# Jun-CEN/Open-World-Semantic-Segmentation

Hardware: AMD Instinct MI355X
Metric: images/sec train-step, DeepLabV3+R101 768x768 bs=16; % HBM & MFMA roofline (higher is better)
Workload: dtype f16x2

## Files before the change

open-world-semantic-segmentation_amd/csrc/bn.hip:

```cpp
#include "common.h"
#include <cstdlib>

namespace {

struct Moments {
    double n, mean, m2;
};
__device__ __forceinline__ void merge(Moments& a, double nb, double meanb, double m2b) {
    if (nb <= 0.0) return;
    const double n = a.n + nb;
    const double d = meanb - a.mean;
    a.mean += d * (nb / n);
    a.m2 += m2b + d * d * (a.n * nb / n);
    a.n = n;
}

constexpr int FIN_CH = 4, FIN_SL = 64;
__device__ __forceinline__ double shfl_xor_f64(double v, int mask) {
    const long long b = __double_as_longlong(v);
    const int lo = __shfl_xor((int)(b & 0xffffffffll), mask), hi = __shfl_xor((int)(b >> 32), mask);
    return __longlong_as_double(((long long)hi << 32) | (unsigned int)lo);
}

__device__ __forceinline__ float h2_words_max(const float* __restrict__ words, float* sh4) {
// ... 1202 lines not shown
#pragma unroll
                for (int t = 0; t < 2; ++t) {
                    const int s = 2 * bx + t - (2 * xo - 1);
                    if (s < 0 || s > 2) continue;
#pragma unroll
                    for (int q = 0; q < 4; ++q) acc[u][t][q] += (((am >> (q * 8)) & 0xffu) == (uint32_t)(r * 3 + s)) ? g[q] : 0.f;
                }
            }
        }
    }
#pragma unroll
    for (int u = 0; u < 2; ++u) {
#pragma unroll
        for (int t = 0; t < 2; ++t) {
            const int yi = 2 * by + u, xi = 2 * bx + t;
            if (yi >= H || xi >= W) continue;
            const uint32_t bits = mask[(((int64_t)b * H + yi) * W + xi) * (C / 4) + cv];
#pragma unroll
            for (int q = 0; q < 4; ++q) acc[u][t][q] = ((bits >> q) & 1u) != 0 ? acc[u][t][q] : 0.f;
        }
    }
}

__device__ __forceinline__ void stem_pixel_grad(const float* __restrict__ dp, const uint8_t* __restrict__ argmax, uint32_t bits, int b,
                                                int yi, int xi, int C, int Ho, int Wo, int cv, float (&acc)[4]) {
#pragma unroll
    for (int q = 0; q < 4; ++q) acc[q] = 0.f;
    const int by = yi >> 1, bx = xi >> 1, u = yi & 1, t = xi & 1;
#pragma unroll
    for (int dyo = 0; dyo < 2; ++dyo) {
        const int yo = by + dyo, r = u + 1 - 2 * dyo;
        if (yo >= Ho || r < 0) continue;
#pragma unroll
        for (int dxo = 0; dxo < 2; ++dxo) {
            const int xo = bx + dxo, sc = t + 1 - 2 * dxo;
            if (xo >= Wo || sc < 0) continue;
            const int64_t o = (((int64_t)b * Ho + yo) * Wo + xo) * C + cv * 4;
            float g[4];
            Vec16<float>::load(dp + o, g);
            const uint32_t am = *reinterpret_cast<const uint32_t*>(argmax + o);
#pragma unroll
            for (int q = 0; q < 4; ++q) acc[q] += (((am >> (q * 8)) & 0xffu) == (uint32_t)(r * 3 + sc)) ? g[q] : 0.f;
        }
    }
#pragma unroll
    for (int q = 0; q < 4; ++q) acc[q] = ((bits >> q) & 1u) != 0 ? acc[q] : 0.f;
}

__global__ __launch_bounds__(256) void stem_bwd_reduce_kernel(
    const float* __restrict__ dp, const uint8_t* __restrict__ argmax, const uint8_t* __restrict__ mask, const float* __restrict__ y,
    const float* __restrict__ save_mean, const float* __restrict__ save_invstd, float* __restrict__ partials, int B, int H, int W,
    int C, int ldy, int Ho, int Wo, int rows_per_block, int chv, int rt, uint32_t* __restrict__ gmax) {
    __shared__ float sh[256 * 2 * 4];
    uint32_t gmx = 0;
    const int NV = C / 4;
    const int64_t M = (int64_t)B * H * W;
    const int col = threadIdx.x % chv, rl = threadIdx.x / chv;
    const int v = blockIdx.y * chv + col;
    const bool active = rl < rt && v < NV;
    float sg[4], sgx[4];
#pragma unroll
    for (int q = 0; q < 4; ++q) { sg[q] = 0.f; sgx[q] = 0.f; }
    if (active) {
        const int c = v * 4;
        float mu[4], is[4];
#pragma unroll
        for (int q = 0; q < 4; ++q) { mu[q] = save_mean[c + q]; is[q] = save_invstd[c + q]; }
        const int64_t r0 = (int64_t)blockIdx.x * rows_per_block;
        const int64_t r1 = min(M, r0 + rows_per_block);
        constexpr int U = 2;
        for (int64_t m0 = r0 + rl; m0 < r1; m0 += (int64_t)rt * U) {
            float g[U][4], yy[U][4];
#pragma unroll
            for (int u = 0; u < U; ++u) {
                const int64_t m = m0 + (int64_t)u * rt;
                if (m < r1) {
                    const int xi = (int)(m % W), yi = (int)((m / W) % H), b = (int)(m / ((int64_t)W * H));
                    Vec16<float>::load(y + m * ldy + c, yy[u]);
                    stem_pixel_grad(dp, argmax, mask[m * NV + v], b, yi, xi, C, Ho, Wo, v, g[u]);
                }
            }
#pragma unroll
            for (int u = 0; u < U; ++u) {
                const int64_t m = m0 + (int64_t)u * rt;
                if (m >= r1) continue;
#pragma unroll
                for (int q = 0; q < 4; ++q) {
                    const float gg = g[u][q];
                    gmx = max(gmx, __float_as_uint(gg) & 0x7fffffffu);
                    sg[q] += gg;
                    sgx[q] += gg * (yy[u][q] - mu[q]) * is[q];
                }
            }
        }
    }
#pragma unroll
    for (int q = 0; q < 4; ++q) {
        sh[(threadIdx.x * 4 + q) * 2] = sg[q];
        sh[(threadIdx.x * 4 + q) * 2 + 1] = sgx[q];
    }
    __syncthreads();
    if (rl == 0 && v < NV) {
        for (int r = 1; r < rt; ++r) {
            const int t = r * chv + col;
// ... 144 lines not shown
#pragma unroll
        for (int q = 0; q < 4; ++q) wr[k][q] = k < K ? w[(int64_t)k * ldw + c + q] : 0.f;
    }
}
template <int KP>
__device__ __forceinline__ void head_load_de(const float* __restrict__ de_row, float (&d)[KP]) {
#pragma unroll
    for (int k = 0; k < KP; k += 4) {
        const float4 t = *reinterpret_cast<const float4*>(de_row + k);
        d[k] = t.x; d[k + 1] = t.y; d[k + 2] = t.z; d[k + 3] = t.w;
    }
}
template <int KP>
__device__ __forceinline__ void head_dz(const float (&d)[KP], const float (&wr)[KP][4], float (&g)[4]) {
#pragma unroll
    for (int q = 0; q < 4; ++q) {
        float a = 0.f;
#pragma unroll
        for (int k = 0; k < KP; ++k) a = fmaf(d[k], wr[k][q], a);
        g[q] = a;
    }
}

template <int KP>
__global__ __launch_bounds__(256) void head_bwd_reduce_kernel(
    const float* __restrict__ de, const float* __restrict__ w, const float* __restrict__ y, const uint8_t* __restrict__ mask,
    const float* __restrict__ save_mean, const float* __restrict__ save_invstd, float* __restrict__ partials, int64_t M, int N,
    int K, int ldde, int ldw, int ldy, int relu, int rows_per_block, int chv, int rt, uint32_t* __restrict__ gmax) {
    __shared__ float sh[256 * 2 * 4];
    uint32_t gmx = 0;
    const int NV = N / 4;
    const int col = threadIdx.x % chv, rl = threadIdx.x / chv;
    const int v = blockIdx.y * chv + col;
    const bool active = rl < rt && v < NV;
    float sg[4], sgx[4];
#pragma unroll
    for (int q = 0; q < 4; ++q) { sg[q] = 0.f; sgx[q] = 0.f; }
    if (active) {
        const int c = v * 4;
        float mu[4], is[4], wr[KP][4];
#pragma unroll
        for (int q = 0; q < 4; ++q) { mu[q] = save_mean[c + q]; is[q] = save_invstd[c + q]; }
        head_load_w<KP>(w, K, ldw, c, wr);
        const int64_t r0 = (int64_t)blockIdx.x * rows_per_block;
        const int64_t r1 = min(M, r0 + rows_per_block);
        constexpr int U = 2;
        for (int64_t m0 = r0 + rl; m0 < r1; m0 += (int64_t)rt * U) {
            float d[U][KP], yy[U][4];
            uint32_t bits[U];
#pragma unroll
            for (int u = 0; u < U; ++u) {
                const int64_t m = m0 + (int64_t)u * rt;
                bits[u] = 0xfu;
                if (m < r1) {
                    head_load_de<KP>(de + m * ldde, d[u]);
// ... 19 lines not shown
    }
#pragma unroll
    for (int q = 0; q < 4; ++q) {
        sh[(threadIdx.x * 4 + q) * 2] = sg[q];
        sh[(threadIdx.x * 4 + q) * 2 + 1] = sgx[q];
    }
    __syncthreads();
    if (rl == 0 && v < NV) {
        for (int r = 1; r < rt; ++r) {
            const int t = r * chv + col;
#pragma unroll
            for (int q = 0; q < 4; ++q) {
                sg[q] += sh[(t * 4 + q) * 2];
                sgx[q] += sh[(t * 4 + q) * 2 + 1];
            }
        }
        float* p = partials + ((int64_t)blockIdx.x * N + v * 4) * 2;
#pragma unroll
        for (int q = 0; q < 4; ++q) { p[2 * q] = sg[q]; p[2 * q + 1] = sgx[q]; }
    }
    if (gmax != nullptr) amax_publish(gmx, gmax);
}

template <int KP, int U, bool PAIR>
__global__ __launch_bounds__(64) void head_bwd_apply_kernel(
    const float* __restrict__ de, const float* __restrict__ w, const float* __restrict__ y, const uint8_t* __restrict__ mask,
    const float* __restrict__ coef, float* __restrict__ dy, int64_t M, int N, int K, int ldde, int ldw, int ldy, int lddy, int relu,
    int CB, int RB, int rows_per_block, _Float16* __restrict__ planes, int64_t plane_stride, int ldp,
    const float* __restrict__ unscale) {
    typedef _Float16 h4 __attribute__((ext_vector_type(4)));
    const float h2s = planes != nullptr ? 1.0f / unscale[0] : 1.0f;
    const int NV = N / 4;
    const int col = threadIdx.x % CB, rl = threadIdx.x / CB;
    const int vcol = blockIdx.y * CB + col;
    if (!(rl < RB && vcol < NV)) return;
    const int c = vcol * 4;
    float cA[4], cB[4], cC[4], cM[4], wr[KP][4];
#pragma unroll
    for (int q = 0; q < 4; ++q) {
        cA[q] = coef[c + q];
        cB[q] = coef[N + c + q];
        cC[q] = coef[2 * N + c + q];
        cM[q] = coef[3 * N + c + q];
    }
    head_load_w<KP>(w, K, ldw, c, wr);
    const int64_t r0 = (int64_t)blockIdx.x * rows_per_block;
    const int64_t r1 = min(M, r0 + rows_per_block);
    for (int64_t m0 = r0 + rl; m0 < r1; m0 += (int64_t)RB * U) {
        float d[U][KP], yy[U][4];
        uint32_t bits[U];
#pragma unroll
        for (int u = 0; u < U; ++u) {
            const int64_t m = m0 + (int64_t)u * RB;
            bits[u] = 0xfu;
            if (m < r1) {
                head_load_de<KP>(de + m * ldde, d[u]);
// ... 44 lines not shown
        return DML_EALIGN;
    if (M >= (1ll << 31)) return DML_EINVAL;
    return 0;
}
}

extern "C" int dml_head_bn_bwd_reduce(const void* de, const float* w, const void* y, const uint8_t* mask, const float* save_mean,
                                      const float* save_invstd, float* partials, int64_t M, int N, int K, int Kp, int ldde, int ldw,
                                      int ldy, int relu, int* nblocks, float* gmax, void* stream) {
    if (const int rc = head_bwd_args(de, w, y, mask, M, N, K, Kp, ldde, ldw, ldy, relu)) return rc;
    if (!save_mean || !save_invstd || !partials || !nblocks) return DML_EINVAL;
    const int NV = N / 4;
    const int chv = NV < RED_COLS ? NV : RED_COLS;
    const int rt = 256 / chv;
    const int col_chunks = (NV + chv - 1) / chv;
    int64_t rpb = (M * col_chunks + 1023) / 1024;
    if (rpb < 4 * rt) rpb = 4 * rt;
    rpb = ((rpb + rt - 1) / rt) * rt;
    const int rb = (int)((M + rpb - 1) / rpb);
    *nblocks = rb;
    const dim3 grid(rb, col_chunks);
    hipStream_t st = static_cast<hipStream_t>(stream);
#define DML_HEAD_REDUCE(KP)                                                                                                       \
    hipLaunchKernelGGL(head_bwd_reduce_kernel<KP>, grid, dim3(256), 0, st, (const float*)de, w, (const float*)y, mask, save_mean, \
                       save_invstd, partials, M, N, K, ldde, ldw, ldy, relu, (int)rpb, chv, rt, reinterpret_cast<uint32_t*>(gmax))
    if (Kp == 8) DML_HEAD_REDUCE(8);
    else if (Kp == 16) DML_HEAD_REDUCE(16);
    else if (Kp == 24) DML_HEAD_REDUCE(24);
    else DML_HEAD_REDUCE(32);
#undef DML_HEAD_REDUCE
    DML_LAUNCH_CHECK();
    return 0;
}

extern "C" int dml_head_bn_bwd_apply(const void* de, const float* w, const void* y, const uint8_t* mask, const float* coef, void* dy,
                                     int64_t M, int N, int K, int Kp, int ldde, int ldw, int ldy, int lddy, int relu, void* planes,
                                     int64_t plane_stride, int32_t ldp, const float* unscale, void* stream) {
    if (const int rc = head_bwd_args(de, w, y, mask, M, N, K, Kp, ldde, ldw, ldy, relu)) return rc;
    if (!coef || (!dy && !planes)) return DML_EINVAL;
    if (dy && ((lddy & 3) || lddy < N || (reinterpret_cast<uintptr_t>(dy) & 15))) return DML_EALIGN;
    if (planes) {
        if (!unscale || plane_stride <= 0 || ldp < N) return DML_EINVAL;
        if ((ldp & 3) || (plane_stride & 3) || (reinterpret_cast<uintptr_t>(planes) & 7)) return DML_EALIGN;
    }
    constexpr int bt = 64;
    const ColGeom g = col_geom(M, N / 4, 2, stream_blocks(M, N, DML_F32), bt);
    const dim3 grid(g.row_blocks, g.col_chunks);
    hipStream_t st = static_cast<hipStream_t>(stream);
    const bool pair = planes && !dy && (N & 7) == 0 && (ldp & 7) == 0 && (plane_stride & 7) == 0 &&
                      (reinterpret_cast<uintptr_t>(planes) & 15) == 0;
#define DML_HEAD_APPLY(KP, PAIR)                                                                                                   \
    hipLaunchKernelGGL((head_bwd_apply_kernel<KP, 2, PAIR>), grid, dim3(bt), 0, st, (const float*)de, w, (const float*)y, mask, coef, \
                       (float*)dy, M, N, K, ldde, ldw, ldy, lddy, relu, g.CB, g.RB, g.rows_per_block,                              \
                       static_cast<_Float16*>(planes), plane_stride, (int)ldp, unscale)
    if (pair) {
        if (Kp == 8) DML_HEAD_APPLY(8, true);
        else if (Kp == 16) DML_HEAD_APPLY(16, true);
        else if (Kp == 24) DML_HEAD_APPLY(24, true);
        else DML_HEAD_APPLY(32, true);
    } else {
        if (Kp == 8) DML_HEAD_APPLY(8, false);
        else if (Kp == 16) DML_HEAD_APPLY(16, false);
        else if (Kp == 24) DML_HEAD_APPLY(24, false);
        else DML_HEAD_APPLY(32, false);
    }
#undef DML_HEAD_APPLY
    DML_LAUNCH_CHECK();
    return 0;
}

namespace {
__global__ __launch_bounds__(256) void h2_bound_kernel(const float* __restrict__ p0, const float* __restrict__ p1,
                                                       const float* __restrict__ p2, const float* __restrict__ invstd, int N,
                                                       float root_count, float mult, const float* __restrict__ words,
                                                       float* __restrict__ work, int bwd) {
    __shared__ float sh[4];
    __shared__ uint32_t shw[4];
// ... 114 lines not shown
```

open-world-semantic-segmentation_amd/csrc/optim_layout.hip:

```cpp
#include "common.h"

namespace {

__global__ __launch_bounds__(256) void sgd_kernel(float* __restrict__ p, const float* __restrict__ g,
                                                  float* __restrict__ v, int64_t n, float lr, float mu, float wd,
                                                  float gscale) {
    const int64_t n4 = n >> 2;
    for (int64_t i = (int64_t)blockIdx.x * blockDim.x + threadIdx.x; i < n4;
         i += (int64_t)gridDim.x * blockDim.x) {
        float4 pp = reinterpret_cast<float4*>(p)[i];
        const float4 gg = reinterpret_cast<const float4*>(g)[i];
        float4 vv = reinterpret_cast<float4*>(v)[i];
        vv.x = mu * vv.x + (gscale * gg.x + wd * pp.x);
        vv.y = mu * vv.y + (gscale * gg.y + wd * pp.y);
        vv.z = mu * vv.z + (gscale * gg.z + wd * pp.z);
        vv.w = mu * vv.w + (gscale * gg.w + wd * pp.w);
        pp.x -= lr * vv.x; pp.y -= lr * vv.y; pp.z -= lr * vv.z; pp.w -= lr * vv.w;
        reinterpret_cast<float4*>(v)[i] = vv;
        reinterpret_cast<float4*>(p)[i] = pp;
    }
    const int64_t base = n4 << 2;
    const int64_t t = base + (int64_t)blockIdx.x * blockDim.x + threadIdx.x;
    if (t < n) {
        const float d = gscale * g[t] + wd * p[t];
// ... 373 lines not shown
    if (!table_device || count <= 0) return DML_EINVAL;
    hipStream_t st = static_cast<hipStream_t>(stream);
    hipLaunchKernelGGL(h2_amax_table_kernel, dim3(H2_TABLE_BLK, count), dim3(256), 0, st, table_device);
    hipLaunchKernelGGL(h2_split_table_kernel, dim3(H2_TABLE_BLK, count), dim3(256), 0, st, table_device);
    DML_LAUNCH_CHECK();
    return 0;
}

namespace {
__global__ __launch_bounds__(256) void pack_input_s2d_kernel(const float* __restrict__ x, float* __restrict__ y, int B, int C, int H, int W) {
    const int H2 = H >> 1, W2 = W >> 1, C4 = 4 * C;
    const int64_t total = (int64_t)B * H2 * W2;
    for (int64_t i = (int64_t)blockIdx.x * blockDim.x + threadIdx.x; i < total; i += (int64_t)gridDim.x * blockDim.x) {
        const int64_t b = i / ((int64_t)H2 * W2);
        const int64_t rem = i - b * H2 * W2;
        const int y2 = (int)(rem / W2), x2 = (int)(rem - (int64_t)y2 * W2);
        float* o = y + i * C4;
        for (int c = 0; c < C; ++c) {
            const float* src = x + ((b * C + c) * H + 2 * y2) * W + 2 * x2;
            o[c] = src[0]; o[C + c] = src[1]; o[2 * C + c] = src[W]; o[3 * C + c] = src[W + 1];
        }
    }
}
template <bool TO_S2D>
__global__ __launch_bounds__(256) void s2d_weights_kernel(float* __restrict__ w, float* __restrict__ w2, int N, int k, int C) {
    const int k2 = (k + 1) / 2, C4 = 4 * C, off = 2 * (((k - 1) / 2 + 1) / 2) - (k - 1) / 2;
    const int total = N * k2 * k2 * C4;
    for (int i = blockIdx.x * blockDim.x + threadIdx.x; i < total; i += gridDim.x * blockDim.x) {
        const int j = i % C4, s2 = (i / C4) % k2, r2 = (i / (C4 * k2)) % k2, n = i / (C4 * k2 * k2);
        const int c = j % C, dx = (j / C) & 1, dy = j / (2 * C);
        const int t = 2 * r2 + dy - off, u = 2 * s2 + dx - off;
        const bool in = t >= 0 && t < k && u >= 0 && u < k;
        const int wi = ((n * k + t) * k + u) * C + c;
        if (TO_S2D) w2[i] = in ? w[wi] : 0.f;
        else if (in) w[wi] += w2[i];
    }
}
}

namespace {
__global__ __launch_bounds__(256) void gather_taps_kernel(const float* __restrict__ src, float* __restrict__ dst, int rows, int taps_src,
                                                          int n, int ntaps, int t0, int t1, int t2, int t3) {
    const int n4 = n >> 2;
    const int64_t total = (int64_t)rows * ntaps * n4;
    for (int64_t i = (int64_t)blockIdx.x * blockDim.x + threadIdx.x; i < total; i += (int64_t)gridDim.x * blockDim.x) {
        const int v = (int)(i % n4), j = (int)((i / n4) % ntaps);
        const int64_t row = i / ((int64_t)n4 * ntaps);
        const int t = j == 0 ? t0 : (j == 1 ? t1 : (j == 2 ? t2 : t3));
        reinterpret_cast<float4*>(dst)[i] = reinterpret_cast<const float4*>(src)[(row * taps_src + t) * n4 + v];
    }
}
}

extern "C" int dml_gather_taps(const float* src, float* dst, int rows, int taps_src, int n, int ntaps, int t0, int t1, int t2, int t3,
                               void* stream) {
    if (!src || !dst || rows <= 0 || taps_src <= 0 || n <= 0 || ntaps <= 0 || ntaps > 4) return DML_EINVAL;
    const int t[4] = {t0, t1, t2, t3};
    for (int j = 0; j < ntaps; ++j)
        if (t[j] < 0 || t[j] >= taps_src) return DML_EINVAL;
    if ((n & 3) || ((reinterpret_cast<uintptr_t>(src) | reinterpret_cast<uintptr_t>(dst)) & 15)) return DML_EALIGN;
    hipLaunchKernelGGL(gather_taps_kernel, dim3(grid_for((int64_t)rows * ntaps * (n >> 2), 256, 256 * 16)), dim3(256), 0,
                       static_cast<hipStream_t>(stream), src, dst, rows, taps_src, n, ntaps, t0, t1, t2, t3);
    DML_LAUNCH_CHECK();
    return 0;
}

extern "C" int dml_pack_input_s2d(const float* x_nchw, float* y, int B, int C, int H, int W, void* stream) {
    if (!x_nchw || !y || B <= 0 || C <= 0 || H <= 0 || W <= 0) return DML_EINVAL;
    if ((H | W) & 1) return DML_EALIGN;
    hipLaunchKernelGGL(pack_input_s2d_kernel, dim3(grid_for((int64_t)B * (H / 2) * (W / 2), 256, 256 * 16)), dim3(256), 0,
                       static_cast<hipStream_t>(stream), x_nchw, y, B, C, H, W);
    DML_LAUNCH_CHECK();
    return 0;
}
extern "C" int dml_s2d_weights(const float* w, float* w2, int N, int k, int C, void* stream) {
    if (!w || !w2 || N <= 0 || C <= 0 || k < 3 || (k & 1) == 0 || (((k - 1) / 2) & 1) == 0) return DML_EINVAL;
    const int k2 = (k + 1) / 2;
    hipLaunchKernelGGL(s2d_weights_kernel<true>, dim3(grid_for((int64_t)N * k2 * k2 * 4 * C, 256)), dim3(256), 0,
                       static_cast<hipStream_t>(stream), const_cast<float*>(w), w2, N, k, C);
    DML_LAUNCH_CHECK();
    return 0;
}
extern "C" int dml_s2d_wgrad(const float* dw2, float* dw, int N, int k, int C, void* stream) {
    if (!dw2 || !dw || N <= 0 || C <= 0 || k < 3 || (k & 1) == 0 || (((k - 1) / 2) & 1) == 0) return DML_EINVAL;
    const int k2 = (k + 1) / 2;
    hipLaunchKernelGGL(s2d_weights_kernel<false>, dim3(grid_for((int64_t)N * k2 * k2 * 4 * C, 256)), dim3(256), 0,
                       static_cast<hipStream_t>(stream), dw, const_cast<float*>(dw2), N, k, C);
    DML_LAUNCH_CHECK();
    return 0;
}

extern "C" int dml_unpad_wgrad(const float* src, float* dst, int N, int RS, int Cm, int Cp, void* stream) {
    if (!src || !dst || Cp < Cm) return DML_EINVAL;
    hipLaunchKernelGGL(unpad_wgrad_kernel, dim3(grid_for((int64_t)N * RS * Cm, 256)), dim3(256), 0,
// ... 63 lines not shown
```

open-world-semantic-segmentation_amd/csrc/pool_resize.hip:

```cpp
#include "common.h"

namespace {

template <typename T>
__global__ __launch_bounds__(256) void maxpool_fwd_kernel(const T* __restrict__ x, T* __restrict__ y,
                                                          uint8_t* __restrict__ argmax, int B, int H, int W,
                                                          int C, int Ho, int Wo) {
    constexpr int V = Vec16<T>::N;
    const int CV = C / V;
    const int64_t total = (int64_t)B * Ho * Wo * CV;
    for (int64_t i = (int64_t)blockIdx.x * blockDim.x + threadIdx.x; i < total;
         i += (int64_t)gridDim.x * blockDim.x) {
        const int cv = (int)(i % CV);
        int64_t p = i / CV;
        const int xo = (int)(p % Wo); p /= Wo;
        const int yo = (int)(p % Ho);
        const int b = (int)(p / Ho);
        float best[V];
        int idx[V];
#pragma unroll
        for (int q = 0; q < V; ++q) { best[q] = -INFINITY; idx[q] = -1; }
#pragma unroll
        for (int r = 0; r < 3; ++r) {
            const int yi = yo * 2 - 1 + r;
// ... 167 lines not shown
         i += (int64_t)gridDim.x * blockDim.x) {
        const int cv = (int)(i % CV);
        int64_t p = i / CV;
        const int X = (int)(p % W); p /= W;
        const int Y = (int)(p % H);
        const int b = (int)(p / H);
        const Lerp ly = src_index(Y, sy, h), lx = src_index(X, sx, w);
        const TI* base = x + (int64_t)b * h * w * ldx + cv * V;
        float o[V];
#pragma unroll
        for (int q = 0; q < V; ++q) {
            const float v00 = Elem<TI>::ld(base + ((int64_t)ly.i0 * w + lx.i0) * ldx + q);
            const float v01 = Elem<TI>::ld(base + ((int64_t)ly.i0 * w + lx.i1) * ldx + q);
            const float v10 = Elem<TI>::ld(base + ((int64_t)ly.i1 * w + lx.i0) * ldx + q);
            const float v11 = Elem<TI>::ld(base + ((int64_t)ly.i1 * w + lx.i1) * ldx + q);
            o[q] = ly.l0 * (lx.l0 * v00 + lx.l1 * v01) + ly.l1 * (lx.l0 * v10 + lx.l1 * v11);
        }
        TO* yp = y + (((int64_t)b * H + Y) * W + X) * ldy + cv * V;
#pragma unroll
        for (int q = 0; q < V; ++q) Elem<TO>::st(yp + q, o[q]);
    }
}

__global__ __launch_bounds__(256) void bilinear_fwd_planes_kernel(const float* __restrict__ x, _Float16* __restrict__ planes,
                                                                  int64_t plane_stride, int ldp, const float* __restrict__ unscale, int B,
                                                                  int h, int w, int H, int W, int C, int ldx, float sy, float sx) {
    typedef _Float16 h4 __attribute__((ext_vector_type(4)));
    const int CV = C / 4;
    const float s = 1.0f / unscale[0];
    const int64_t total = (int64_t)B * H * W * CV;
    for (int64_t i = (int64_t)blockIdx.x * blockDim.x + threadIdx.x; i < total; i += (int64_t)gridDim.x * blockDim.x) {
        const int cv = (int)(i % CV);
        int64_t p = i / CV;
        const int X = (int)(p % W); p /= W;
        const int Y = (int)(p % H);
        const int b = (int)(p / H);
        const Lerp ly = src_index(Y, sy, h), lx = src_index(X, sx, w);
        const float* base = x + (int64_t)b * h * w * ldx + cv * 4;
        const float4 v00 = *reinterpret_cast<const float4*>(base + ((int64_t)ly.i0 * w + lx.i0) * ldx);
        const float4 v01 = *reinterpret_cast<const float4*>(base + ((int64_t)ly.i0 * w + lx.i1) * ldx);
        const float4 v10 = *reinterpret_cast<const float4*>(base + ((int64_t)ly.i1 * w + lx.i0) * ldx);
        const float4 v11 = *reinterpret_cast<const float4*>(base + ((int64_t)ly.i1 * w + lx.i1) * ldx);
        const float a00[4] = {v00.x, v00.y, v00.z, v00.w}, a01[4] = {v01.x, v01.y, v01.z, v01.w};
        const float a10[4] = {v10.x, v10.y, v10.z, v10.w}, a11[4] = {v11.x, v11.y, v11.z, v11.w};
        h4 hi, lo;
#pragma unroll
        for (int q = 0; q < 4; ++q) {
            const float o = ly.l0 * (lx.l0 * a00[q] + lx.l1 * a01[q]) + ly.l1 * (lx.l0 * a10[q] + lx.l1 * a11[q]);
            const float xs = o * s;
            const _Float16 hh = (_Float16)xs;
            hi[q] = hh;
            lo[q] = (_Float16)(xs - (float)hh);
        }
        _Float16* yp = planes + (((int64_t)b * H + Y) * W + X) * ldp + cv * 4;
        *reinterpret_cast<h4*>(yp) = hi;
        *reinterpret_cast<h4*>(yp + plane_stride) = lo;
    }
}

template <typename TI, typename TO>
__global__ __launch_bounds__(256) void bilinear_bwd_kernel(const TI* __restrict__ dy, TO* __restrict__ dx, int B,
                                                           int h, int w, int H, int W, int C, int lddy, int lddx,
                                                           float sy, float sx) {
    constexpr int V = 4;
    const int CV = C / V;
    const int64_t total = (int64_t)B * h * w * CV;
    for (int64_t i = (int64_t)blockIdx.x * blockDim.x + threadIdx.x; i < total;
         i += (int64_t)gridDim.x * blockDim.x) {
        const int cv = (int)(i % CV);
        int64_t p = i / CV;
        const int xs = (int)(p % w); p /= w;
        const int ys = (int)(p % h);
        const int b = (int)(p / h);
        const int Y0 = max(0, (int)floorf(((float)ys - 0.5f) / sy - 0.5f) - 1);
        const int Y1 = min(H - 1, (int)ceilf(((float)ys + 1.5f) / sy - 0.5f) + 1);
        const int X0 = max(0, (int)floorf(((float)xs - 0.5f) / sx - 0.5f) - 1);
        const int X1 = min(W - 1, (int)ceilf(((float)xs + 1.5f) / sx - 0.5f) + 1);
        float acc[V] = {0.f, 0.f, 0.f, 0.f};
        for (int Y = Y0; Y <= Y1; ++Y) {
            const Lerp ly = src_index(Y, sy, h);
            const float wy = (ly.i0 == ys ? ly.l0 : 0.f) + (ly.i1 == ys ? ly.l1 : 0.f);
            if (wy == 0.f) continue;
            for (int X = X0; X <= X1; ++X) {
                const Lerp lx = src_index(X, sx, w);
                const float wx = (lx.i0 == xs ? lx.l0 : 0.f) + (lx.i1 == xs ? lx.l1 : 0.f);
                if (wx == 0.f) continue;
                const TI* g = dy + (((int64_t)b * H + Y) * W + X) * lddy + cv * V;
#pragma unroll
                for (int q = 0; q < V; ++q) acc[q] += wy * wx * Elem<TI>::ld(g + q);
            }
        }
        TO* o = dx + (((int64_t)b * h + ys) * w + xs) * lddx + cv * V;
#pragma unroll
        for (int q = 0; q < V; ++q) Elem<TO>::st(o + q, acc[q]);
    }
}

__global__ __launch_bounds__(256) void bilinear_fwd_bf16v_kernel(const bf16_t* __restrict__ x, bf16_t* __restrict__ y, int B,
                                                                 int h, int w, int H, int W, int C, int ldx, int ldy,
                                                                 float sy, float sx) {
    const int CV = C / 8;
    const int64_t total = (int64_t)B * H * W * CV;
    const int64_t i = (int64_t)blockIdx.x * blockDim.x + threadIdx.x;
    if (i >= total) return;
    const int cv = (int)(i % CV);
    int64_t p = i / CV;
    const int X = (int)(p % W); p /= W;
    const int Y = (int)(p % H);
    const int b = (int)(p / H);
    const Lerp ly = src_index(Y, sy, h), lx = src_index(X, sx, w);
    const bf16_t* base = x + (int64_t)b * h * w * ldx + cv * 8;
    float v00[8], v01[8], v10[8], v11[8], o[8];
    Vec16<bf16_t>::load(base + ((int64_t)ly.i0 * w + lx.i0) * ldx, v00);
    Vec16<bf16_t>::load(base + ((int64_t)ly.i0 * w + lx.i1) * ldx, v01);
    Vec16<bf16_t>::load(base + ((int64_t)ly.i1 * w + lx.i0) * ldx, v10);
    Vec16<bf16_t>::load(base + ((int64_t)ly.i1 * w + lx.i1) * ldx, v11);
#pragma unroll
    for (int q = 0; q < 8; ++q) o[q] = ly.l0 * (lx.l0 * v00[q] + lx.l1 * v01[q]) + ly.l1 * (lx.l0 * v10[q] + lx.l1 * v11[q]);
    Vec16<bf16_t>::store(y + (((int64_t)b * H + Y) * W + X) * ldy + cv * 8, o);
}
// ... 207 lines not shown
template <bool BWD>
static int launch_bilinear(const void* src, void* dst, int B, int h, int w, int H, int W, int C, int ld_src,
                           int ld_dst, int dtype, int in_f32, int out_f32, void* stream) {
    if (!src || !dst || B <= 0 || h <= 0 || w <= 0 || H <= 0 || W <= 0) return DML_EINVAL;
    if (C % 4) return DML_EALIGN;
    const float sy = (float)h / (float)H, sx = (float)w / (float)W;
    const int64_t items = BWD ? (int64_t)B * h * w * (C / 4) : (int64_t)B * H * W * (C / 4);
    const int grid = grid_for(items, 256, 256 * 16);
    hipStream_t st = static_cast<hipStream_t>(stream);
    const bool fi = in_f32 || dtype == DML_F32, fo = out_f32 || dtype == DML_F32;
    if (!fi && !fo && C % 8 == 0 && ld_src % 8 == 0 && ld_dst % 8 == 0 && (reinterpret_cast<uintptr_t>(src) & 15) == 0 &&
        (reinterpret_cast<uintptr_t>(dst) & 15) == 0) {
        const int64_t it8 = BWD ? (int64_t)B * h * w * (C / 8) : (int64_t)B * H * W * (C / 8);
        const dim3 g8((unsigned)((it8 + 255) / 256));
        if (BWD)
            hipLaunchKernelGGL(bilinear_bwd_bf16v_kernel, g8, dim3(256), 0, st, (const bf16_t*)src, (bf16_t*)dst, B, h, w, H, W, C,
                               ld_src, ld_dst, sy, sx);
        else
            hipLaunchKernelGGL(bilinear_fwd_bf16v_kernel, g8, dim3(256), 0, st, (const bf16_t*)src, (bf16_t*)dst, B, h, w, H, W, C,
                               ld_src, ld_dst, sy, sx);
        DML_LAUNCH_CHECK();
        return 0;
    }
#define GO(TI, TO)                                                                                           \
    do {                                                                                                     \
        if (BWD)                                                                                             \
            hipLaunchKernelGGL((bilinear_bwd_kernel<TI, TO>), dim3(grid), dim3(256), 0, st, (const TI*)src,  \
                               (TO*)dst, B, h, w, H, W, C, ld_src, ld_dst, sy, sx);                          \
        else                                                                                                 \
            hipLaunchKernelGGL((bilinear_fwd_kernel<TI, TO>), dim3(grid), dim3(256), 0, st, (const TI*)src,  \
                               (TO*)dst, B, h, w, H, W, C, ld_src, ld_dst, sy, sx);                          \
    } while (0)
    if (fi && fo) GO(float, float);
    else if (fi) GO(float, bf16_t);
    else if (fo) GO(bf16_t, float);
    else GO(bf16_t, bf16_t);
#undef GO
    DML_LAUNCH_CHECK();
    return 0;
}

extern "C" int dml_bilinear_fwd(const void* x, void* y, int B, int h, int w, int H, int W, int C, int ldx, int ldy,
                                int dtype, int in_f32, int out_f32, void* stream) {
    return launch_bilinear<false>(x, y, B, h, w, H, W, C, ldx, ldy, dtype, in_f32, out_f32, stream);
}
extern "C" int dml_bilinear_fwd_planes(const float* x, void* planes, int64_t plane_stride, int ldp, const float* unscale, int B, int h,
                                       int w, int H, int W, int C, int ldx, void* stream) {
    if (!x || !planes || !unscale || B <= 0 || h <= 0 || w <= 0 || H <= 0 || W <= 0 || C <= 0 || plane_stride <= 0) return DML_EINVAL;
    if ((C & 3) || (ldx & 3) || (ldp & 3) || (plane_stride & 3) || ldp < C || ldx < C || (reinterpret_cast<uintptr_t>(x) & 15) ||
        (reinterpret_cast<uintptr_t>(planes) & 7))
        return DML_EALIGN;
    const float sy = (float)h / (float)H, sx = (float)w / (float)W;
    const int64_t total = (int64_t)B * H * W * (C / 4);
    hipLaunchKernelGGL(bilinear_fwd_planes_kernel, dim3(grid_for(total, 256, 256 * 32)), dim3(256), 0, static_cast<hipStream_t>(stream), x,
                       static_cast<_Float16*>(planes), plane_stride, ldp, unscale, B, h, w, H, W, C, ldx, sy, sx);
    DML_LAUNCH_CHECK();
    return 0;
}
extern "C" int dml_bilinear_bwd(const void* dy, void* dx, int B, int h, int w, int H, int W, int C, int lddy,
                                int lddx, int dtype, int in_f32, int out_f32, void* stream) {
    return launch_bilinear<true>(dy, dx, B, h, w, H, W, C, lddy, lddx, dtype, in_f32, out_f32, stream);
}

namespace {
__device__ __forceinline__ int bin_lo(int i, int n, int s) { return (int)(((int64_t)i * n) / s); }
__device__ __forceinline__ int bin_hi(int i, int n, int s) { return (int)((((int64_t)(i + 1)) * n + s - 1) / s); }

template <typename T>
__global__ __launch_bounds__(256) void adaptive_pool_partial_kernel(const T* __restrict__ x, float* __restrict__ part, int H,
                                                                    int W, int C, int ldx, int S, int RS) {
    constexpr int V = Vec16<T>::N;
    const int cv = blockIdx.y * 256 + threadIdx.x;
    if (cv * V >= C) return;
    const int rs = blockIdx.x % RS, bin = blockIdx.x / RS;
    const int j = bin % S, i = (bin / S) % S, b = bin / (S * S);
    const int y0 = bin_lo(i, H, S), y1 = bin_hi(i, H, S), x0 = bin_lo(j, W, S), x1 = bin_hi(j, W, S);
    const int rows = (y1 - y0 + RS - 1) / RS;
    const int ya = y0 + rs * rows, yb = min(y1, ya + rows);
// ... 140 lines not shown
```

Measured before the change: 217.5.

## Rework stem/head BN backward, s2d packing, and bilinear resize kernels

Several unrelated kernel changes land together. The stem BN backward reduce now issues all four pooled-gradient loads unconditionally and updates pixel coordinates incrementally instead of using 64-bit div/mod. The head backward kernels get wave-uniform row-index specializations. Input space-to-depth packing is staged through LDS for coalesced writes. The bilinear backward path gains a dedicated 4x-upsample gather kernel with XCD-aware block remapping, and the fp16 planes forward uses 8-wide vectors with 32-bit indexing. Each targets memory or indexing overhead, at the cost of more code paths and extra redundant loads at borders.

```diff
diff --git a/open-world-semantic-segmentation_amd/csrc/bn.hip b/open-world-semantic-segmentation_amd/csrc/bn.hip
--- a/open-world-semantic-segmentation_amd/csrc/bn.hip
+++ b/open-world-semantic-segmentation_amd/csrc/bn.hip
@@ -1248,26 +1248,36 @@
     }
 }
 
-__device__ __forceinline__ void stem_pixel_grad(const float* __restrict__ dp, const uint8_t* __restrict__ argmax, uint32_t bits, int b,
-                                                int yi, int xi, int C, int Ho, int Wo, int cv, float (&acc)[4]) {
-#pragma unroll
-    for (int q = 0; q < 4; ++q) acc[q] = 0.f;
+struct StemPixel {
+    float4 g[4];
+    uint32_t am[4];
+    int tap[4];
+};
+__device__ __forceinline__ void stem_pixel_load(const float* __restrict__ dp, const uint8_t* __restrict__ argmax, int b, int yi, int xi,
+                                                int C, int Ho, int Wo, int cv, StemPixel& px) {
     const int by = yi >> 1, bx = xi >> 1, u = yi & 1, t = xi & 1;
 #pragma unroll
     for (int dyo = 0; dyo < 2; ++dyo) {
         const int yo = by + dyo, r = u + 1 - 2 * dyo;
-        if (yo >= Ho || r < 0) continue;
 #pragma unroll
         for (int dxo = 0; dxo < 2; ++dxo) {
-            const int xo = bx + dxo, sc = t + 1 - 2 * dxo;
-            if (xo >= Wo || sc < 0) continue;
-            const int64_t o = (((int64_t)b * Ho + yo) * Wo + xo) * C + cv * 4;
-            float g[4];
-            Vec16<float>::load(dp + o, g);
-            const uint32_t am = *reinterpret_cast<const uint32_t*>(argmax + o);
-#pragma unroll
-            for (int q = 0; q < 4; ++q) acc[q] += (((am >> (q * 8)) & 0xffu) == (uint32_t)(r * 3 + sc)) ? g[q] : 0.f;
-        }
+            const int xo = bx + dxo, sc = t + 1 - 2 * dxo, k = 2 * dyo + dxo;
+            const bool have = yo < Ho && r >= 0 && xo < Wo && sc >= 0;
+            px.tap[k] = have ? r * 3 + sc : 256;
+            const int64_t o = (((int64_t)b * Ho + (have ? yo : by)) * Wo + (have ? xo : bx)) * C + cv * 4;
+            px.g[k] = *reinterpret_cast<const float4*>(dp + o);
+            px.am[k] = *reinterpret_cast<const uint32_t*>(argmax + o);
+        }
+    }
+}
+__device__ __forceinline__ void stem_pixel_sum(const StemPixel& px, uint32_t bits, float (&acc)[4]) {
+#pragma unroll
+    for (int q = 0; q < 4; ++q) acc[q] = 0.f;
+#pragma unroll
+    for (int k = 0; k < 4; ++k) {
+        const float g[4] = {px.g[k].x, px.g[k].y, px.g[k].z, px.g[k].w};
+#pragma unroll
+        for (int q = 0; q < 4; ++q) acc[q] += (((px.am[k] >> (q * 8)) & 0xffu) == (uint32_t)px.tap[k]) ? g[q] : 0.f;
     }
 #pragma unroll
     for (int q = 0; q < 4; ++q) acc[q] = ((bits >> q) & 1u) != 0 ? acc[q] : 0.f;
@@ -1295,17 +1305,37 @@
         const int64_t r0 = (int64_t)blockIdx.x * rows_per_block;
         const int64_t r1 = min(M, r0 + rows_per_block);
         constexpr int U = 2;
+        const int dxs = rt % W, dys = (rt / W) % H, dbs = rt / W / H;
+        int xi = 0, yi = 0, b = 0;
+        if (r0 + rl < r1) {
+            const uint32_t m = (uint32_t)(r0 + rl), row = m / (uint32_t)W;
+            xi = (int)(m - row * (uint32_t)W);
+            b = (int)(row / (uint32_t)H);
+            yi = (int)(row - (uint32_t)b * (uint32_t)H);
+        }
         for (int64_t m0 = r0 + rl; m0 < r1; m0 += (int64_t)rt * U) {
             float g[U][4], yy[U][4];
+            StemPixel px[U];
+            uint32_t bits[U];
 #pragma unroll
             for (int u = 0; u < U; ++u) {
                 const int64_t m = m0 + (int64_t)u * rt;
                 if (m < r1) {
-                    const int xi = (int)(m % W), yi = (int)((m / W) % H), b = (int)(m / ((int64_t)W * H));
                     Vec16<float>::load(y + m * ldy + c, yy[u]);
-                    stem_pixel_grad(dp, argmax, mask[m * NV + v], b, yi, xi, C, Ho, Wo, v, g[u]);
+                    bits[u] = mask[m * NV + v];
+                    stem_pixel_load(dp, argmax, b, yi, xi, C, Ho, Wo, v, px[u]);
+                    xi += dxs;
+                    const int cx = xi >= W ? 1 : 0;
+                    xi -= cx ? W : 0;
+                    yi += dys + cx;
+                    const int cy = yi >= H ? 1 : 0;
+                    yi -= cy ? H : 0;
+                    b += dbs + cy;
                 }
             }
+#pragma unroll
+            for (int u = 0; u < U; ++u)
+                if (m0 + (int64_t)u * rt < r1) stem_pixel_sum(px[u], bits[u], g[u]);
 #pragma unroll
             for (int u = 0; u < U; ++u) {
                 const int64_t m = m0 + (int64_t)u * rt;
@@ -1496,7 +1526,7 @@
     }
 }
 
-template <int KP>
+template <int KP, bool UNI>
 __global__ __launch_bounds__(256) void head_bwd_reduce_kernel(
     const float* __restrict__ de, const float* __restrict__ w, const float* __restrict__ y, const uint8_t* __restrict__ mask,
     const float* __restrict__ save_mean, const float* __restrict__ save_invstd, float* __restrict__ partials, int64_t M, int N,
@@ -1504,7 +1534,8 @@
     __shared__ float sh[256 * 2 * 4];
     uint32_t gmx = 0;
     const int NV = N / 4;
-    const int col = threadIdx.x % chv, rl = threadIdx.x / chv;
+    const int col = threadIdx.x % chv;
+    const int rl = UNI ? __builtin_amdgcn_readfirstlane((int)(threadIdx.x / chv)) : (int)(threadIdx.x / chv);
     const int v = blockIdx.y * chv + col;
     const bool active = rl < rt && v < NV;
     float sg[4], sgx[4];
@@ -1570,7 +1601,7 @@
     if (gmax != nullptr) amax_publish(gmx, gmax);
 }
 
-template <int KP, int U, bool PAIR>
+template <int KP, int U, bool PAIR, bool UNI>
 __global__ __launch_bounds__(64) void head_bwd_apply_kernel(
     const float* __restrict__ de, const float* __restrict__ w, const float* __restrict__ y, const uint8_t* __restrict__ mask,
     const float* __restrict__ coef, float* __restrict__ dy, int64_t M, int N, int K, int ldde, int ldw, int ldy, int lddy, int relu,
@@ -1579,7 +1610,8 @@
     typedef _Float16 h4 __attribute__((ext_vector_type(4)));
     const float h2s = planes != nullptr ? 1.0f / unscale[0] : 1.0f;
     const int NV = N / 4;
-    const int col = threadIdx.x % CB, rl = threadIdx.x / CB;
+    const int col = threadIdx.x % CB;
+    const int rl = UNI ? 0 : (int)(threadIdx.x / CB);
     const int vcol = blockIdx.y * CB + col;
     if (!(rl < RB && vcol < NV)) return;
     const int c = vcol * 4;
@@ -1670,8 +1702,16 @@
     const dim3 grid(rb, col_chunks);
     hipStream_t st = static_cast<hipStream_t>(stream);
 #define DML_HEAD_REDUCE(KP)                                                                                                       \
-    hipLaunchKernelGGL(head_bwd_reduce_kernel<KP>, grid, dim3(256), 0, st, (const float*)de, w, (const float*)y, mask, save_mean, \
-                       save_invstd, partials, M, N, K, ldde, ldw, ldy, relu, (int)rpb, chv, rt, reinterpret_cast<uint32_t*>(gmax))
+    do {                                                                                                                          \
+        if (chv == 64)                                                                                                            \
+            hipLaunchKernelGGL((head_bwd_reduce_kernel<KP, true>), grid, dim3(256), 0, st, (const float*)de, w, (const float*)y,  \
+                               mask, save_mean, save_invstd, partials, M, N, K, ldde, ldw, ldy, relu, (int)rpb, chv, rt,          \
+                               reinterpret_cast<uint32_t*>(gmax));                                                                \
+        else                                                                                                                      \
+            hipLaunchKernelGGL((head_bwd_reduce_kernel<KP, false>), grid, dim3(256), 0, st, (const float*)de, w, (const float*)y, \
+                               mask, save_mean, save_invstd, partials, M, N, K, ldde, ldw, ldy, relu, (int)rpb, chv, rt,          \
+                               reinterpret_cast<uint32_t*>(gmax));                                                                \
+    } while (0)
     if (Kp == 8) DML_HEAD_REDUCE(8);
     else if (Kp == 16) DML_HEAD_REDUCE(16);
     else if (Kp == 24) DML_HEAD_REDUCE(24);
@@ -1698,9 +1738,16 @@
     const bool pair = planes && !dy && (N & 7) == 0 && (ldp & 7) == 0 && (plane_stride & 7) == 0 &&
                       (reinterpret_cast<uintptr_t>(planes) & 15) == 0;
 #define DML_HEAD_APPLY(KP, PAIR)                                                                                                   \
-    hipLaunchKernelGGL((head_bwd_apply_kernel<KP, 2, PAIR>), grid, dim3(bt), 0, st, (const float*)de, w, (const float*)y, mask, coef, \
-                       (float*)dy, M, N, K, ldde, ldw, ldy, lddy, relu, g.CB, g.RB, g.rows_per_block,                              \
-                       static_cast<_Float16*>(planes), plane_stride, (int)ldp, unscale)
+    do {                                                                                                                           \
+        if (g.CB == bt)                                                                                                            \
+            hipLaunchKernelGGL((head_bwd_apply_kernel<KP, 2, PAIR, true>), grid, dim3(bt), 0, st, (const float*)de, w,             \
+                               (const float*)y, mask, coef, (float*)dy, M, N, K, ldde, ldw, ldy, lddy, relu, g.CB, g.RB,           \
+                               g.rows_per_block, static_cast<_Float16*>(planes), plane_stride, (int)ldp, unscale);                 \
+        else                                                                                                                       \
+            hipLaunchKernelGGL((head_bwd_apply_kernel<KP, 2, PAIR, false>), grid, dim3(bt), 0, st, (const float*)de, w,            \
+                               (const float*)y, mask, coef, (float*)dy, M, N, K, ldde, ldw, ldy, lddy, relu, g.CB, g.RB,           \
+                               g.rows_per_block, static_cast<_Float16*>(planes), plane_stride, (int)ldp, unscale);                 \
+    } while (0)
     if (pair) {
         if (Kp == 8) DML_HEAD_APPLY(8, true);
         else if (Kp == 16) DML_HEAD_APPLY(16, true);
diff --git a/open-world-semantic-segmentation_amd/csrc/optim_layout.hip b/open-world-semantic-segmentation_amd/csrc/optim_layout.hip
--- a/open-world-semantic-segmentation_amd/csrc/optim_layout.hip
+++ b/open-world-semantic-segmentation_amd/csrc/optim_layout.hip
@@ -419,6 +419,35 @@
         }
     }
 }
+constexpr int S2D_TP = 256;
+template <bool PAIRS>
+__global__ __launch_bounds__(256) void pack_input_s2d_rows_kernel(const float* __restrict__ x, float* __restrict__ y, int B, int C, int H,
+                                                                  int W) {
+    extern __shared__ __attribute__((aligned(16))) float s2d_tile[];
+    const int H2 = H >> 1, W2 = W >> 1, C4 = 4 * C;
+    const int64_t total = (int64_t)B * H2 * W2;
+    const int64_t i0 = (int64_t)blockIdx.x * S2D_TP;
+    const int n = (int)min((int64_t)S2D_TP, total - i0);
+    for (int it = threadIdx.x; it < 2 * C * S2D_TP; it += 256) {
+        const int p = it % S2D_TP, cd = it / S2D_TP, c = cd >> 1, dy = cd & 1;
+        if (p >= n) continue;
+        const int64_t i = i0 + p, b = i / ((int64_t)H2 * W2), rem = i - b * H2 * W2;
+        const int y2 = (int)(rem / W2), x2 = (int)(rem - (int64_t)y2 * W2);
+        const float* src = x + ((b * C + c) * H + 2 * y2 + dy) * W + 2 * x2;
+        float v0, v1;
+        if (PAIRS) {
+            const float2 v = *reinterpret_cast<const float2*>(src);
+            v0 = v.x; v1 = v.y;
+        } else {
+            v0 = src[0]; v1 = src[1];
+        }
+        s2d_tile[p * C4 + (2 * dy) * C + c] = v0;
+        s2d_tile[p * C4 + (2 * dy + 1) * C + c] = v1;
+    }
+    __syncthreads();
+    float4* o = reinterpret_cast<float4*>(y + i0 * C4);
+    for (int v = threadIdx.x; v < n * C; v += 256) o[v] = reinterpret_cast<const float4*>(s2d_tile)[v];
+}
 template <bool TO_S2D>
 __global__ __launch_bounds__(256) void s2d_weights_kernel(float* __restrict__ w, float* __restrict__ w2, int N, int k, int C) {
     const int k2 = (k + 1) / 2, C4 = 4 * C, off = 2 * (((k - 1) / 2 + 1) / 2) - (k - 1) / 2;
@@ -465,8 +494,19 @@
 extern "C" int dml_pack_input_s2d(const float* x_nchw, float* y, int B, int C, int H, int W, void* stream) {
     if (!x_nchw || !y || B <= 0 || C <= 0 || H <= 0 || W <= 0) return DML_EINVAL;
     if ((H | W) & 1) return DML_EALIGN;
-    hipLaunchKernelGGL(pack_input_s2d_kernel, dim3(grid_for((int64_t)B * (H / 2) * (W / 2), 256, 256 * 16)), dim3(256), 0,
-                       static_cast<hipStream_t>(stream), x_nchw, y, B, C, H, W);
+    const int64_t tiles = ((int64_t)B * (H / 2) * (W / 2) + S2D_TP - 1) / S2D_TP;
+    if (C <= 4 && tiles <= 0x7fffffff && (reinterpret_cast<uintptr_t>(y) & 15) == 0 && (reinterpret_cast<uintptr_t>(x_nchw) & 3) == 0) {
+        const size_t lds = (size_t)S2D_TP * 4 * C * sizeof(float);
+        if ((reinterpret_cast<uintptr_t>(x_nchw) & 7) == 0)
+            hipLaunchKernelGGL(pack_input_s2d_rows_kernel<true>, dim3((unsigned)tiles), dim3(256), lds, static_cast<hipStream_t>(stream),
+                               x_nchw, y, B, C, H, W);
+        else
+            hipLaunchKernelGGL(pack_input_s2d_rows_kernel<false>, dim3((unsigned)tiles), dim3(256), lds, static_cast<hipStream_t>(stream),
+                               x_nchw, y, B, C, H, W);
+    } else {
+        hipLaunchKernelGGL(pack_input_s2d_kernel, dim3(grid_for((int64_t)B * (H / 2) * (W / 2), 256, 256 * 16)), dim3(256), 0,
+                           static_cast<hipStream_t>(stream), x_nchw, y, B, C, H, W);
+    }
     DML_LAUNCH_CHECK();
     return 0;
 }
diff --git a/open-world-semantic-segmentation_amd/csrc/pool_resize.hip b/open-world-semantic-segmentation_amd/csrc/pool_resize.hip
--- a/open-world-semantic-segmentation_amd/csrc/pool_resize.hip
+++ b/open-world-semantic-segmentation_amd/csrc/pool_resize.hip
@@ -213,39 +213,49 @@
     }
 }
 
+template <int V, typename IT>
 __global__ __launch_bounds__(256) void bilinear_fwd_planes_kernel(const float* __restrict__ x, _Float16* __restrict__ planes,
                                                                   int64_t plane_stride, int ldp, const float* __restrict__ unscale, int B,
                                                                   int h, int w, int H, int W, int C, int ldx, float sy, float sx) {
-    typedef _Float16 h4 __attribute__((ext_vector_type(4)));
-    const int CV = C / 4;
+    typedef _Float16 hv __attribute__((ext_vector_type(V)));
+    const int CV = C / V;
     const float s = 1.0f / unscale[0];
-    const int64_t total = (int64_t)B * H * W * CV;
-    for (int64_t i = (int64_t)blockIdx.x * blockDim.x + threadIdx.x; i < total; i += (int64_t)gridDim.x * blockDim.x) {
-        const int cv = (int)(i % CV);
-        int64_t p = i / CV;
-        const int X = (int)(p % W); p /= W;
-        const int Y = (int)(p % H);
-        const int b = (int)(p / H);
+    const IT total = (IT)((int64_t)B * H * W * CV);
+    for (IT i = (IT)blockIdx.x * blockDim.x + threadIdx.x; i < total; i += (IT)gridDim.x * blockDim.x) {
+        IT p = i / (IT)CV;
+        const int cv = (int)(i - p * (IT)CV);
+        IT pw = p / (IT)W;
+        const int X = (int)(p - pw * (IT)W);
+        const int b = (int)(pw / (IT)H);
+        const int Y = (int)(pw - (IT)b * (IT)H);
         const Lerp ly = src_index(Y, sy, h), lx = src_index(X, sx, w);
-        const float* base = x + (int64_t)b * h * w * ldx + cv * 4;
-        const float4 v00 = *reinterpret_cast<const float4*>(base + ((int64_t)ly.i0 * w + lx.i0) * ldx);
-        const float4 v01 = *reinterpret_cast<const float4*>(base + ((int64_t)ly.i0 * w + lx.i1) * ldx);
-        const float4 v10 = *reinterpret_cast<const float4*>(base + ((int64_t)ly.i1 * w + lx.i0) * ldx);
-        const float4 v11 = *reinterpret_cast<const float4*>(base + ((int64_t)ly.i1 * w + lx.i1) * ldx);
-        const float a00[4] = {v00.x, v00.y, v00.z, v00.w}, a01[4] = {v01.x, v01.y, v01.z, v01.w};
-        const float a10[4] = {v10.x, v10.y, v10.z, v10.w}, a11[4] = {v11.x, v11.y, v11.z, v11.w};
-        h4 hi, lo;
-#pragma unroll
-        for (int q = 0; q < 4; ++q) {
+        const float* base = x + (int64_t)b * h * w * ldx + cv * V;
+        const float* p00 = base + ((int64_t)ly.i0 * w + lx.i0) * ldx;
+        const float* p01 = base + ((int64_t)ly.i0 * w + lx.i1) * ldx;
+        const float* p10 = base + ((int64_t)ly.i1 * w + lx.i0) * ldx;
+        const float* p11 = base + ((int64_t)ly.i1 * w + lx.i1) * ldx;
+        float a00[V], a01[V], a10[V], a11[V];
+#pragma unroll
+        for (int u = 0; u < V; u += 4) {
+            const float4 v00 = *reinterpret_cast<const float4*>(p00 + u), v01 = *reinterpret_cast<const float4*>(p01 + u);
+            const float4 v10 = *reinterpret_cast<const float4*>(p10 + u), v11 = *reinterpret_cast<const float4*>(p11 + u);
+            a00[u] = v00.x; a00[u + 1] = v00.y; a00[u + 2] = v00.z; a00[u + 3] = v00.w;
+            a01[u] = v01.x; a01[u + 1] = v01.y; a01[u + 2] = v01.z; a01[u + 3] = v01.w;
+            a10[u] = v10.x; a10[u + 1] = v10.y; a10[u + 2] = v10.z; a10[u + 3] = v10.w;
+            a11[u] = v11.x; a11[u + 1] = v11.y; a11[u + 2] = v11.z; a11[u + 3] = v11.w;
+        }
+        hv hi, lo;
+#pragma unroll
+        for (int q = 0; q < V; ++q) {
             const float o = ly.l0 * (lx.l0 * a00[q] + lx.l1 * a01[q]) + ly.l1 * (lx.l0 * a10[q] + lx.l1 * a11[q]);
             const float xs = o * s;
             const _Float16 hh = (_Float16)xs;
             hi[q] = hh;
             lo[q] = (_Float16)(xs - (float)hh);
         }
-        _Float16* yp = planes + (((int64_t)b * H + Y) * W + X) * ldp + cv * 4;
-        *reinterpret_cast<h4*>(yp) = hi;
-        *reinterpret_cast<h4*>(yp + plane_stride) = lo;
+        _Float16* yp = planes + (((int64_t)b * H + Y) * W + X) * ldp + cv * V;
+        *reinterpret_cast<hv*>(yp) = hi;
+        *reinterpret_cast<hv*>(yp + plane_stride) = lo;
     }
 }
 
@@ -287,6 +297,94 @@
     }
 }
 
+__device__ __forceinline__ float bwd_x4_weight(int D, int s, float scale, int in, int Dn) {
+    if (s >= in || (unsigned)D >= (unsigned)Dn) return 0.f;
+    const Lerp l = src_index(D, scale, in);
+    return (l.i0 == s ? l.l0 : 0.f) + (l.i1 == s ? l.l1 : 0.f);
+}
+template <bool CHECK>
+__device__ __forceinline__ void bwd_x4_window(const float* __restrict__ base, int Yb, int Xb, int H, int W, int lddy,
+                                              const float (&wy)[2][8], const float (&wx)[2][8], float4 (&acc)[2][2]) {
+#pragma unroll
+    for (int r = 0; r < 12; ++r) {
+        const int Y = Yb + r;
+        if (CHECK && (unsigned)Y >= (unsigned)H) continue;
+        const float* row = base + (int64_t)Y * W * lddy;
+        float4 g[12];
+#pragma unroll
+        for (int c = 0; c < 12; ++c)
+            g[c] = *reinterpret_cast<const float4*>(row + (int64_t)(CHECK ? min(max(Xb + c, 0), W - 1) : Xb + c) * lddy);
+#pragma unroll
+        for (int j = 0; j < 2; ++j) {
+            if (r < 4 * j || r >= 4 * j + 8) continue;
+            const float a = wy[j][r - 4 * j];
+            if (CHECK && a == 0.f) continue;
+#pragma unroll
+            for (int c = 0; c < 12; ++c)
+#pragma unroll
+                for (int k = 0; k < 2; ++k) {
+                    if (c < 4 * k || c >= 4 * k + 8) continue;
+                    const float bb = wx[k][c - 4 * k];
+                    if (CHECK && bb == 0.f) continue;
+                    acc[j][k].x += a * bb * g[c].x;
+                    acc[j][k].y += a * bb * g[c].y;
+                    acc[j][k].z += a * bb * g[c].z;
+                    acc[j][k].w += a * bb * g[c].w;
+                }
+        }
+    }
+}
+template <bool UNI>
+__device__ __forceinline__ float bwd_x4_uniform(float v) {
+    return UNI ? __int_as_float(__builtin_amdgcn_readfirstlane(__float_as_int(v))) : v;
+}
+template <bool UNI>
+__global__ __launch_bounds__(256) void bilinear_bwd_x4_kernel(const float* __restrict__ dy, float* __restrict__ dx, int B, int h, int w,
+                                                              int H, int W, int C, int lddy, int lddx, float sy, float sx,
+                                                              int ngy, int ngx) {
+    const int nb = (int)gridDim.x, q8 = nb >> 3, r8 = nb & 7, xcd = (int)blockIdx.x & 7;
+    const int64_t bid = (int64_t)xcd * q8 + min(xcd, r8) + ((int)blockIdx.x >> 3);
+    const int CV = C >> 2;
+    const int64_t i = bid * 256 + threadIdx.x;
+    const int cv = (int)(i % CV);
+    int64_t t = i / CV;
+    if (UNI) t = __builtin_amdgcn_readfirstlane((int)t);
+    const int quad = (int)(t & 3); t >>= 2;
+    const int gx = (int)(t % ngx); t /= ngx;
+    const int gy = (int)(t % ngy);
+    const int64_t b = t / ngy;
+    const int ys0 = 2 * (2 * gy + (quad >> 1)), xs0 = 2 * (2 * gx + (quad & 1));
+    if (b >= B || ys0 >= h || xs0 >= w) return;
+    const int Yb = 4 * ys0 - 2, Xb = 4 * xs0 - 2;
+    float wy[2][8], wx[2][8];
+#pragma unroll
+    for (int j = 0; j < 2; ++j)
+#pragma unroll
+        for (int r = 0; r < 8; ++r) {
+            wy[j][r] = bwd_x4_uniform<UNI>(bwd_x4_weight(Yb + 4 * j + r, ys0 + j, sy, h, H));
+            wx[j][r] = bwd_x4_uniform<UNI>(bwd_x4_weight(Xb + 4 * j + r, xs0 + j, sx, w, W));
+        }
+    float4 acc[2][2];
+#pragma unroll
+    for (int j = 0; j < 2; ++j)
+#pragma unroll
+        for (int k = 0; k < 2; ++k) acc[j][k] = make_float4(0.f, 0.f, 0.f, 0.f);
+    const float* base = dy + b * H * W * lddy + cv * 4;
+    bool inner = true;
+#pragma unroll
+    for (int j = 0; j < 2; ++j)
+#pragma unroll
+        for (int r = 0; r < 8; ++r) inner = inner && wy[j][r] != 0.f && wx[j][r] != 0.f;
+    if (inner) bwd_x4_window<false>(base, Yb, Xb, H, W, lddy, wy, wx, acc);
+    else bwd_x4_window<true>(base, Yb, Xb, H, W, lddy, wy, wx, acc);
+#pragma unroll
+    for (int j = 0; j < 2; ++j)
+#pragma unroll
+        for (int k = 0; k < 2; ++k)
+            if (ys0 + j < h && xs0 + k < w)
+                *reinterpret_cast<float4*>(dx + ((b * h + ys0 + j) * w + xs0 + k) * lddx + cv * 4) = acc[j][k];
+}
+
 __global__ __launch_bounds__(256) void bilinear_fwd_bf16v_kernel(const bf16_t* __restrict__ x, bf16_t* __restrict__ y, int B,
                                                                  int h, int w, int H, int W, int C, int ldx, int ldy,
                                                                  float sy, float sx) {
@@ -540,7 +638,22 @@
         DML_LAUNCH_CHECK();
         return 0;
     }
-#define GO(TI, TO)                                                                                           \
+    if (BWD && fi && fo && H == 4 * (int64_t)h && W == 4 * (int64_t)w && C % 16 == 0 && ld_src % 4 == 0 && ld_dst % 4 == 0 &&
+        (reinterpret_cast<uintptr_t>(src) & 15) == 0 && (reinterpret_cast<uintptr_t>(dst) & 15) == 0) {
+        const int ngy = ((h + 1) / 2 + 1) / 2, ngx = ((w + 1) / 2 + 1) / 2;
+        const int64_t tiles = (int64_t)B * ngy * ngx * 4, blocks = (tiles * (C / 4) + 255) / 256;
+        if (blocks <= 0x7fffffff && tiles <= 0x7fffffff) {
+            if (C % 256 == 0)
+                hipLaunchKernelGGL(bilinear_bwd_x4_kernel<true>, dim3((unsigned)blocks), dim3(256), 0, st, (const float*)src, (float*)dst,
+                                   B, h, w, H, W, C, ld_src, ld_dst, sy, sx, ngy, ngx);
+            else
+                hipLaunchKernelGGL(bilinear_bwd_x4_kernel<false>, dim3((unsigned)blocks), dim3(256), 0, st, (const float*)src, (float*)dst,
+                                   B, h, w, H, W, C, ld_src, ld_dst, sy, sx, ngy, ngx);
+            DML_LAUNCH_CHECK();
+            return 0;
+        }
+    }
+#define GO(TI, TO)                                                                                        \
     do {                                                                                                     \
         if (BWD)                                                                                             \
             hipLaunchKernelGGL((bilinear_bwd_kernel<TI, TO>), dim3(grid), dim3(256), 0, st, (const TI*)src,  \
@@ -569,9 +682,18 @@
         (reinterpret_cast<uintptr_t>(planes) & 7))
         return DML_EALIGN;
     const float sy = (float)h / (float)H, sx = (float)w / (float)W;
-    const int64_t total = (int64_t)B * H * W * (C / 4);
-    hipLaunchKernelGGL(bilinear_fwd_planes_kernel, dim3(grid_for(total, 256, 256 * 32)), dim3(256), 0, static_cast<hipStream_t>(stream), x,
-                       static_cast<_Float16*>(planes), plane_stride, ldp, unscale, B, h, w, H, W, C, ldx, sy, sx);
+    const int64_t total8 = (int64_t)B * H * W * (C / 8);
+    if ((C & 7) == 0 && (ldp & 7) == 0 && (plane_stride & 7) == 0 && (reinterpret_cast<uintptr_t>(planes) & 15) == 0 &&
+        total8 < (1ll << 31)) {
+        hipLaunchKernelGGL((bilinear_fwd_planes_kernel<8, uint32_t>), dim3(grid_for(total8, 256, 256 * 32)), dim3(256), 0,
+                           static_cast<hipStream_t>(stream), x, static_cast<_Float16*>(planes), plane_stride, ldp, unscale, B, h, w, H, W,
+                           C, ldx, sy, sx);
+    } else {
+        const int64_t total = (int64_t)B * H * W * (C / 4);
+        hipLaunchKernelGGL((bilinear_fwd_planes_kernel<4, int64_t>), dim3(grid_for(total, 256, 256 * 32)), dim3(256), 0,
+                           static_cast<hipStream_t>(stream), x, static_cast<_Float16*>(planes), plane_stride, ldp, unscale, B, h, w, H, W,
+                           C, ldx, sy, sx);
+    }
     DML_LAUNCH_CHECK();
     return 0;
 }
```

Measured after the change: 218.8, median of 6. No clear change (+0.6%).
